# ligengen/EgoGen

Measured on AMD Instinct MI355X. Metric: PPO env-steps/sec (512 parallel SMPL-X agents), higher is better.
Workload: dtype f32 (blend GEMM: shape/template columns as 2-term bf16 splits, pose correctives as one fp16 product, fp32 accumulate); PPO update products on 2-term bf16 splits; rollout policy layers on 2-term bf16 splits

## Files before the change

egogen_amd/_lib.py:

```python
from __future__ import annotations

import ctypes as C
import os

_HERE = os.path.dirname(os.path.abspath(__file__))
LIB_PATH = os.path.join(_HERE, "libegogen_hip.so")

c_float_p = C.POINTER(C.c_float)
c_int_p = C.POINTER(C.c_int32)


class EgxError(RuntimeError):
    pass


class BodyModelHost(C.Structure):
    _fields_ = [
        ("num_verts", C.c_int),
        ("v_template_host", C.c_void_p), ("shapedirs_host", C.c_void_p), ("posedirs_host", C.c_void_p),
        ("J_regressor_host", C.c_void_p), ("parents_host", C.c_void_p), ("lbs_weights_host", C.c_void_p),
        ("hand_comps_l_host", C.c_void_p), ("hand_comps_r_host", C.c_void_p),
        ("hand_mean_l_host", C.c_void_p), ("hand_mean_r_host", C.c_void_p),
        ("extra_vids_host", C.c_void_p), ("lmk_vids_host", C.c_void_p), ("lmk_bary_host", C.c_void_p),
        ("num_markers", C.c_int), ("marker_vids_host", C.c_void_p),
# ... 220 lines not shown
    "egx_sample_action": (C.c_int, [C.c_void_p, C.c_void_p, C.c_void_p, C.c_float, C.c_float, C.c_int, C.c_int, C.c_void_p,
                                    C.c_void_p, C.c_void_p]),
    "egx_gae": (C.c_int, [C.c_void_p, C.c_void_p, C.c_void_p, C.c_int, C.c_int, C.c_double, C.c_double, C.c_void_p,
                          C.c_void_p, C.c_void_p]),
    "egx_ppo_loss": (C.c_int, [C.c_void_p] * 9 + [C.c_float] * 6 + [C.c_int] + [C.c_void_p] * 5),
    "egx_gru_pointwise_bwd": (C.c_int, [C.c_void_p, C.c_void_p, C.c_void_p, C.c_void_p, C.c_int, C.c_int, C.c_void_p, C.c_void_p,
                                        C.c_void_p, C.c_void_p]),
    "egx_ppo_loss_packed": (C.c_int, [C.c_void_p] * 8 + [C.c_float] * 6 + [C.c_int] + [C.c_void_p] * 4),
    "egx_lbs_set_blend_mode": (C.c_int, [C.c_int]),
    "egx_lbs_get_blend_mode": (C.c_int, []),
    "egx_lbs_set_wave_tile": (C.c_int, [C.c_int]),
    "egx_lbs_get_wave_tile": (C.c_int, []),
    "egx_lbs_set_fix_queue_capacity": (C.c_int, [C.c_int]),
    "egx_lbs_fix_stats": (C.c_int, [C.c_void_p, C.c_void_p, C.c_int, C.POINTER(C.c_int32)]),
    "egx_gather_rows": (C.c_int, [C.c_void_p, C.c_int, C.c_int, C.c_void_p, C.c_void_p, C.c_void_p, C.c_void_p]),
    "egx_adv_stats": (C.c_int, [C.c_void_p, C.c_int, C.c_void_p, C.c_void_p]),
    "egx_track_episode": (C.c_int, [C.c_void_p, C.c_void_p, C.c_int, C.c_void_p, C.c_void_p, C.c_void_p, C.c_void_p]),
    "egx_rollout_store": (C.c_int, [C.c_void_p] * 6 + [C.c_int] + [C.c_void_p] * 10),
    "egx_adamw_workspace_floats": (C.c_size_t, []),
    "egx_adamw_clip_step": (C.c_int, [C.c_void_p, C.c_void_p, C.c_void_p, C.c_void_p, C.c_size_t, C.c_size_t, C.c_float] + [C.c_double] * 5 +
                            [C.c_void_p, C.c_void_p, C.c_void_p]),
    "egx_policy_set_precision": (C.c_int, [C.c_int]),
    "egx_policy_get_precision": (C.c_int, []),
    "egx_act_fwd": (C.c_int, [C.c_void_p, C.c_void_p, C.c_void_p, C.c_int, C.c_int, C.c_int, C.c_float, C.c_void_p]),
    "egx_act_bwd_colsum": (C.c_int, [C.c_void_p, C.c_void_p, C.c_void_p, C.c_void_p, C.c_int, C.c_int, C.c_int, C.c_float,
                                     C.c_void_p]),
    "egx_profile_next_lbs": (C.c_int, [C.c_void_p, C.c_void_p]),
    "egx_event_create": (C.c_int, [C.POINTER(C.c_void_p)]),
    "egx_event_destroy": (C.c_int, [C.c_void_p]),
    "egx_event_elapsed_ms": (C.c_int, [C.c_void_p, C.c_void_p, C.POINTER(C.c_float)]),
    "egx_policy_train_create": (C.c_int, [C.POINTER(PolicyWeights), C.POINTER(PolicyGrads), C.c_int, C.POINTER(C.c_void_p)]),
    "egx_policy_train_destroy": (None, [C.c_void_p]),
    "egx_policy_train_refresh": (C.c_int, [C.c_void_p, C.c_void_p]),
    "egx_policy_train_packed": (C.c_int, [C.c_void_p, C.POINTER(PolicyPacked3)]),
    "egx_policy_train_bind": (C.c_int, [C.c_void_p, C.c_void_p, C.c_void_p]),
    "egx_policy_train_step": (C.c_int, [C.c_void_p] * 9 + [C.c_float] * 6 + [C.c_void_p, C.c_void_p]),
    "egx_policy_train_step_heads": (C.c_int, [C.c_void_p] * 9 + [C.c_float] * 6 + [C.c_void_p, C.c_void_p]),
    "egx_policy_train_step_encoders": (C.c_int, [C.c_void_p, C.c_void_p]),
    "egx_policy_train_set_precision": (C.c_int, [C.c_void_p, C.c_int]),
    "egx_policy_train_dense3_launches": (C.c_int, [C.c_void_p]),
    "egx_policy_train_head": (C.c_int, [C.c_void_p, C.POINTER(UpdateHead), C.c_void_p]),
    "egx_policy_train_step_cursor": (C.c_int, [C.c_void_p, C.POINTER(UpdateHead), C.c_void_p] + [C.c_float] * 6 + [C.c_void_p]),
    "egx_policy_train_step_heads_cursor": (C.c_int, [C.c_void_p, C.POINTER(UpdateHead), C.c_void_p] + [C.c_float] * 6 + [C.c_void_p]),
    "egx_adamw_clip_step_cursor": (C.c_int, [C.c_void_p, C.c_void_p, C.c_void_p, C.c_void_p, C.c_size_t, C.c_size_t, C.c_float] +
                                   [C.c_double] * 5 + [C.c_void_p, C.c_void_p, C.c_void_p, C.c_void_p]),
    "egx_policy_train_bind_flat": (C.c_int, [C.c_void_p, C.c_void_p, C.c_size_t]),
# ... 57 lines not shown
```

egogen_amd/csrc/body_model.hip:

```cpp
#include <algorithm>
#include <atomic>
#include <cstdlib>

#include "egx_sdf.h"
#include "lbs_pack.h"

static thread_local hipEvent_t g_prof_start = nullptr, g_prof_stop = nullptr;
extern "C" int egx_profile_next_lbs(void* start_event, void* stop_event) {
  g_prof_start = static_cast<hipEvent_t>(start_event);
  g_prof_stop = static_cast<hipEvent_t>(stop_event);
  return EGX_OK;
}

namespace {
constexpr int BODY_PAD = 256;
}

__global__ void egx_gather_kernel(const float* __restrict__ picked, int B, int NP, int M,
                                  const int* __restrict__ marker_slot, const int* __restrict__ extra_slot,
                                  const int* __restrict__ lmk_slot, const float* __restrict__ lmk_bary,
                                  float* __restrict__ out_joints, float* __restrict__ out_markers) {
  const int b = blockIdx.x;
  const float* pk = picked + (size_t)b * NP * 3;
  for (int i = threadIdx.x; i < M + NEXTRA + NLMK; i += blockDim.x) {
    if (i < M) {
      if (out_markers) {
        const float* s = pk + marker_slot[i] * 3;
        float* o = out_markers + ((size_t)b * M + i) * 3;
        o[0] = s[0]; o[1] = s[1]; o[2] = s[2];
      }
    } else if (out_joints) {
      float* o = out_joints + ((size_t)b * EGX_NUM_JOINTS_OUT + NJ + (i - M)) * 3;
      if (i < M + NEXTRA) {
        const float* s = pk + extra_slot[i - M] * 3;
        o[0] = s[0]; o[1] = s[1]; o[2] = s[2];
      } else {
        const int l = i - M - NEXTRA;
        float acc[3] = {0.f, 0.f, 0.f};
        for (int k = 0; k < 3; ++k) {
          const float* s = pk + lmk_slot[l * 3 + k] * 3;
          const float w = lmk_bary[l * 3 + k];
          acc[0] += s[0] * w; acc[1] += s[1] * w; acc[2] += s[2] * w;
        }
        o[0] = acc[0]; o[1] = acc[1]; o[2] = acc[2];
      }
    }
  }
}

extern "C" int egx_body_model_create(const egx_body_model_host* d, egx_body_model** out) {
  EGX_REQUIRE(d && out, "null argument");
  LbsPacked p;
  if (int rc = lbs_pack_model(d, &p)) return rc;
  auto* m = new egx_body_model();
  static_cast<LbsModelDims&>(*m) = p;
  auto u16 = [](bf16x8** dptr) { return reinterpret_cast<unsigned short**>(dptr); };
  int rc = EGX_OK;
  if ((rc = egx_upload(&m->cull_E, p.cull_E)) || (rc = egx_upload(&m->cull_D0, p.cull_D0)) || (rc = egx_upload(u16(&m->dirs3), p.dirs3)) ||
      (rc = egx_upload(u16(&m->dirs4), p.dirs4)) || (rc = egx_upload(u16(&m->skinW), p.skinW)) || (rc = egx_upload(&m->skin_ks_off, p.skin_ks_off)) ||
      (rc = egx_upload(&m->dirs_rm, p.dirs_rm)) || (rc = egx_upload(&m->vorig, p.perm)) || (rc = egx_upload(&m->pick_tiles, p.pick_tiles)) ||
      (rc = egx_upload(&m->sdf_tiles, p.sdf_tiles)) || (rc = egx_upload(&m->dirs, p.dirs)) || (rc = egx_upload(&m->tj_off, p.tj_off)) ||
      (rc = egx_upload(&m->tj_idx, p.tj_idx)) || (rc = egx_upload(&m->tj_w, p.tj_w)) || (rc = egx_upload(&m->pick_slot, p.pick_slot)) ||
      (rc = egx_upload(&m->vflags, p.vflags)) || (rc = egx_upload(&m->pc, p.pc)) || (rc = egx_upload(&m->marker_slot, p.marker_slot)) ||
      (rc = egx_upload(&m->extra_slot, p.extra_slot)) || (rc = egx_upload(&m->lmk_slot, p.lmk_slot)) ||
      (rc = egx_upload(&m->lmk_bary, p.lmk_bary))) {
    egx_body_model_destroy(m);
    return rc;
  }
  *out = m;
  return EGX_OK;
}
// ... 211 lines not shown
  int* order = cull ? reinterpret_cast<int*>(ws + wl.order) : nullptr;
  int* flags = reinterpret_cast<int*>(ws + wl.flags);
  int* items = reinterpret_cast<int*>(ws + wl.items);
  int* counts = reinterpret_cast<int*>(ws + wl.counts);
  float* fvec = cull ? reinterpret_cast<float*>(ws + wl.fvec) : nullptr;
  float* jpos = cull ? reinterpret_cast<float*>(ws + wl.jpos) : nullptr;
  if (cull) lbs_launch_cull_order(m, xb, R0, T0, sd, mips, B, fpa, nbg_all, order, flags, counts, stream);
  const SdfSceneDev* scene_tab = ms ? set->table : nullptr;
  const int n_scenes = ms ? set->S : 0;
  LbsPoseArgs a;
  a.pc = m->pc; a.xb = xb; a.betas = betas; a.B = B; a.fpa = fpa; a.A4 = A4; a.out_joints = out_joints; a.joints_ld = EGX_NUM_JOINTS_OUT;
  if (split3) a.feat3 = reinterpret_cast<unsigned short*>(feat); else a.feat = feat;
  a.template_lo_feat = (split3 && mode >= 2) ? 1.f : 0.f;
  a.feat4 = (split3 && mode == 3) ? feat4 : nullptr;
  a.zero_counts = sdf ? out_pene_count : nullptr;
  a.agent_of_slot = order; a.fvec = fvec; a.jpos = jpos; a.Bp = (int)wl.Bp;
  a.fix_e = fix ? reinterpret_cast<float*>(ws + wl.fix_e) : nullptr;
  a.skinB = fix ? reinterpret_cast<unsigned short*>(ws + wl.skinB) : nullptr;
  a.fix_stats = reinterpret_cast<int*>(ws + wl.fix_stats); a.cinit = reinterpret_cast<f32x4*>(ws + wl.cinit);
  a.R0 = R0; a.T0 = T0; a.sdf = sd; a.scenes = scene_tab; a.agent_scene = agent_scene; a.n_scenes = n_scenes;
  lbs_launch_pose(ms, stream, a);
  if (cull)
    lbs_launch_cull_items(m, fvec, jpos, (int)wl.Bp, order, B, fpa, nbg_all, R0, T0, sd, mips, flags, items, wl.items_stride, counts, stream);
  if (out_verts || need_picks || sdf) {
    LbsParams p;
    p.dirs = m->dirs; p.tj_off = m->tj_off; p.tj_idx = m->tj_idx; p.tj_w = m->tj_w; p.pick_slot = m->pick_slot;
    p.dirs3 = m->dirs3; p.feat3 = reinterpret_cast<const bf16x8*>(feat);
    p.dirs4 = m->dirs4; p.feat4 = reinterpret_cast<const bf16x8*>(feat4);
    p.vorig = m->vorig;
    p.vflags = m->vflags; p.feat = reinterpret_cast<const f32x4*>(feat); p.A4 = A4; p.xb = xb;
    p.B = B; p.V = m->V; p.NVT = m->NVT; p.NW = m->NW; p.NP = m->NP; p.fpa = fpa;
    p.nbg = egx_ceil_div(B, BODY_PAD);
#ifdef EGX_LBS_DEVELOPMENT
    {
      const char* e = getenv("EGX_LBS_DBG");
      p.dbg = e ? atoi(e) : 0;
    }
#else
    p.dbg = 0;
#endif
    p.verts = out_verts; p.picked = picked; p.R0 = R0; p.T0 = T0; p.pene = out_pene_count;
    p.agent_of_slot = order; p.items = cull ? items : nullptr; p.item_counts = counts; p.items_stride = wl.items_stride;
    p.tiles = out_verts ? nullptr : (sdf ? m->sdf_tiles : m->pick_tiles);
    p.n_tiles = out_verts ? m->NVT : (sdf ? m->n_sdf_tiles : m->n_pick_tiles);
    p.n_precise = sdf ? (m->sdf_lead_picks ? m->n_pick_tiles : m->n_sdf_tiles) : m->n_pick_tiles;
#ifdef EGX_LBS_DEVELOPMENT
    if (const char* e = getenv("EGX_LBS_PRECISE")) p.n_precise = atoi(e);
#endif
    p.sdf = sd;
    p.fix_e = reinterpret_cast<const float*>(ws + wl.fix_e);
    p.fix_stats = reinterpret_cast<int*>(ws + wl.fix_stats);
    p.skinW = m->skinW; p.skin_ks_off = m->skin_ks_off;
    p.fixq = reinterpret_cast<int2*>(ws + wl.fixq); p.fixq_cap = g_fixq_cap.load() > 0 ? g_fixq_cap.load() : LBS_FIXQ_CAP;
    p.dirs_rm = m->dirs_rm; p.pc = m->pc; p.betas = betas;
    p.skinB = reinterpret_cast<const bf16x8*>(ws + wl.skinB); p.cinit = reinterpret_cast<const f32x4*>(ws + wl.cinit);
    p.sdf_aux = ms ? nullptr : aux;
    p.scenes = scene_tab; p.agent_scene = agent_scene; p.n_scenes = n_scenes;
    p.bg_block = 3;
#ifdef EGX_LBS_DEVELOPMENT
    if (const char* e = getenv("EGX_LBS_BG_BLOCK")) p.bg_block = atoi(e);
#endif
    hipEvent_t ev0 = g_prof_start, ev1 = g_prof_stop;
    g_prof_start = g_prof_stop = nullptr;
    if (ev0) EGX_HIP_CHECK(hipEventRecord(ev0, stream));
    if (int rc = split3 ? lbs_launch_fused3(p, mode, sdf != nullptr, ms, wave_tile(), stream) : lbs_launch_fused(p, sdf != nullptr, ms, stream))
      return rc;
    if (fix) lbs_launch_fix(p, ms, stream);
    if (ev1) EGX_HIP_CHECK(hipEventRecord(ev1, stream));
  }
  if (need_picks)
    hipLaunchKernelGGL(egx_gather_kernel, dim3(B), dim3(256), 0, stream, picked, B, m->NP, m->M, m->marker_slot,
                       m->extra_slot, m->lmk_slot, m->lmk_bary, out_joints, out_markers);
  EGX_HIP_CHECK(hipGetLastError());
  return EGX_OK;
}

extern "C" int egx_lbs_forward(const egx_body_model* m, const float* xb, const float* betas, int B, int fpa,
                               float* out_verts, float* out_joints, float* out_markers, const egx_sdf_grid* sdf,
                               const float* R0, const float* T0, int32_t* out_pene_count, void* workspace,
                               size_t workspace_bytes, void* stream) {
  return lbs_forward_launch(m, xb, betas, B, fpa, out_verts, out_joints, out_markers, sdf, nullptr, nullptr, R0, T0, out_pene_count,
                            workspace, workspace_bytes, stream);
}

extern "C" int egx_lbs_forward_scenes(const egx_body_model* m, const float* xb, const float* betas, int B, int fpa,
                                      float* out_verts, float* out_joints, float* out_markers, const egx_sdf_scene_set* scenes,
                                      const int32_t* agent_scene, const float* R0, const float* T0, int32_t* out_pene_count,
                                      void* workspace, size_t workspace_bytes, void* stream) {
  EGX_REQUIRE(scenes && agent_scene && out_pene_count, "a scene-set call needs the set, agent_scene and out_pene_count");
  if (scenes->S == 1) {
    if (int rc = lbs_forward_launch(m, xb, betas, B, fpa, out_verts, out_joints, out_markers, &scenes->dims, nullptr, nullptr, R0, T0,
                                    out_pene_count, workspace, workspace_bytes, stream))
      return rc;
    hipLaunchKernelGGL(egx_lbs_scene_mark_kernel, dim3(egx_ceil_div(B, 256)), dim3(256), 0, static_cast<hipStream_t>(stream), agent_scene,
                       1, B, fpa, out_pene_count);
// ... 7 lines not shown
```

egogen_amd/csrc/egx_common.h:

```cpp
#pragma once
#include <hip/hip_runtime.h>
#include <stdint.h>
#include <stdio.h>
#include <string>
#include <vector>

#include "../../include/egogen_hip.h"

typedef float f32x16 __attribute__((ext_vector_type(16)));
typedef float f32x4 __attribute__((ext_vector_type(4)));
typedef short bf16x8 __attribute__((ext_vector_type(8)));
__host__ __device__ inline unsigned short egx_bf16_rne(float x) {
  union { float f; unsigned u; } c;
  c.f = x;
  if ((c.u & 0x7fffffffu) > 0x7f800000u) return (unsigned short)((c.u >> 16) | 0x40u);
  return (unsigned short)((c.u + 0x7fffu + ((c.u >> 16) & 1u)) >> 16);
}
__host__ __device__ inline float egx_bf16_to_f32(unsigned short h) {
  union { float f; unsigned u; } c;
  c.u = (unsigned)h << 16;
  return c.f;
}


void egx_set_error(const std::string& msg);

#define EGX_HIP_CHECK(expr)                                                                   \
  do {                                                                                        \
    hipError_t _e = (expr);                                                                   \
    if (_e != hipSuccess) {                                                                   \
      egx_set_error(std::string(#expr) + ": " + hipGetErrorString(_e));                       \
      return EGX_ERR_HIP;                                                                     \
    }                                                                                         \
  } while (0)

#define EGX_REQUIRE(cond, msg)                                                                \
  do {                                                                                        \
    if (!(cond)) {                                                                            \
      egx_set_error(std::string("argument check failed: ") + #cond + " - " + (msg));          \
      return EGX_ERR_ARG;                                                                     \
    }                                                                                         \
  } while (0)

static inline int egx_ceil_div(int a, int b) { return (a + b - 1) / b; }
static inline size_t egx_align_up(size_t x, size_t a) { return (x + a - 1) / a * a; }

template <typename T>
static int egx_upload(T** dptr, const std::vector<T>& h) {
// ... 18 lines not shown
```

egogen_amd/csrc/egx_nets.h:

```cpp
#pragma once
#include "egx_common.h"
#include "egx_frame.h"

struct EgxSeg {
  const float* p;
  int w, ld;
};

int egx_launch_linear(hipStream_t st, int M, int N, const EgxSeg* segs, int nseg, const float* W, const float* b,
                      int act, float slope, const float* res, int ldr, float* out, int ldo);
int egx_launch_gru_pointwise(hipStream_t st, const float* gi, const float* gh, const float* hprev, int ldh, float* hout,
                             int ldo, int M, int H);
int egx_launch_cont6d_to_aa(hipStream_t st, const float* xb6, int n, float* out, int ldo);
int egx_launch_posenc(hipStream_t st, const float* dist, const float* time, int A, float* out);

void egx_launch_frame_scan(hipStream_t st, float* y, const float* x_last, int x_ld, int A, int width, int T);

struct D3Pack {
  const float* src;
  int R, K, ld, col0;
  void* dst;
  int S_total, s0;
  int transpose = 0;
};
void egx_launch_pack3(hipStream_t st, const D3Pack* jobs, int njobs);

struct D3Plain {
  const bf16x8* A = nullptr;
  int SA = 0, sa0 = 0;
  const bf16x8* B = nullptr;
  int S = 0;
  const float* bias = nullptr;
  const float* res = nullptr;
  int ldr = 0;
  float* out = nullptr;
  int ldo = 0;
  bf16x8* out3 = nullptr;
  int S3 = 0, s30 = 0;
  int M = 0, N = 0, act = 0;
  float slope = 0.f;
  int batches = 1;
  size_t batch_strideA = 0, batch_stride3 = 0;
  int batch_rows_out = 0;
  int prec = 0;
  float* out_act = nullptr;
  int ldact = 0;
  const float* dact = nullptr;
  int lddact = 0, dact_code = 0;
// ... 135 lines not shown
```

egogen_amd/csrc/lbs.h:

```cpp
#pragma once
#include <mutex>

#include "egx_common.h"
#include "egx_sdf.h"

namespace {

constexpr int NJ = EGX_NUM_JOINTS;
constexpr int KACT = 10 + 51 * 9;
constexpr int KDIM = EGX_BLEND_K;
constexpr int KSTEPS = KDIM / 2;
constexpr int KGROUPS = KSTEPS / 4;
static_assert(KGROUPS >= 2, "the operand ring preloads two k-groups");
constexpr int KS3 = 30;
__host__ __device__ inline void egx_bf16_split3(float x, unsigned short* h) {
  h[0] = egx_bf16_rne(x);
  const float r1 = x - egx_bf16_to_f32(h[0]);
  h[1] = egx_bf16_rne(r1);
  const float r2 = r1 - egx_bf16_to_f32(h[1]);
  h[2] = egx_bf16_rne(r2);
}
constexpr int M4_BASE_PIECES = 96, M4_FEAT_PIECES = 32;
constexpr int M4_FKS = 4;
__host__ __device__ inline int egx_m4_feat_piece(int s, int pl) { return s == 0 ? pl : (s <= 28 ? s + 1 : 30 + pl); }
// ... 226 lines not shown
struct LbsPoseArgs {
  const PoseConsts* pc = nullptr;
  const float *xb = nullptr, *betas = nullptr, *R0 = nullptr, *T0 = nullptr;
  int B = 0, fpa = 0, joints_ld = 0, Bp = 0;
  float *feat = nullptr, *out_joints = nullptr, *fvec = nullptr, *jpos = nullptr, *fix_e = nullptr;
  unsigned short *feat3 = nullptr, *feat4 = nullptr, *skinB = nullptr;
  f32x4 *A4 = nullptr, *cinit = nullptr;
  int *zero_counts = nullptr, *fix_stats = nullptr;
  const int* agent_of_slot = nullptr;
  float template_lo_feat = 0.f;
  SdfDev sdf = {};
  const SdfSceneDev* scenes = nullptr;
  const int* agent_scene = nullptr;
  int n_scenes = 0;
};
void lbs_launch_pose(bool ms, hipStream_t stream, const LbsPoseArgs& a);
void lbs_launch_cull_order(const egx_body_model* m, const float* xb, const float* R0, const float* T0, const SdfDev& sd, const float* mips,
                           int B, int fpa, int nbg_all, int* order, int* flags, int* counts, hipStream_t stream);
void lbs_launch_cull_items(const egx_body_model* m, const float* fvec, const float* jpos, int Bp, const int* order, int B, int fpa,
                           int nbg_all, const float* R0, const float* T0, const SdfDev& sd, const float* mips, int* flags, int* items,
                           int items_stride, int* counts, hipStream_t stream);
int lbs_launch_fused(const LbsParams& p, bool do_sdf, bool ms, hipStream_t stream);
int lbs_launch_fused3(const LbsParams& p, int mode, bool do_sdf, bool ms, int forced_tile, hipStream_t stream);
void lbs_launch_fix(const LbsParams& p, bool ms, hipStream_t stream);
```

egogen_amd/csrc/lbs_fix.hip:

```cpp
#include "lbs_epilogue.h"

constexpr int LBS_FIX_BLOCKS = 1024;
static_assert((LBS_FIX_BLOCKS * 4) % LBS_FIX_NQ == 0, "waves of the fix-up kernel per sub-queue");
template <bool MS>
__global__ __launch_bounds__(256) void egx_lbs_fix_kernel(LbsParams p) {
  const int lane = threadIdx.x & 63;
  const int wave = blockIdx.x * 4 + (threadIdx.x >> 6), n_waves = gridDim.x * 4;
  const int sq = wave % LBS_FIX_NQ;
  const int count = min(p.fix_stats[LBS_FIX_CNT0 + 32 * sq], p.fixq_cap);
  for (int i = wave / LBS_FIX_NQ; i < count; i += n_waves / LBS_FIX_NQ) {
    const int2 e = p.fixq[(size_t)sq * p.fixq_cap + i];
    if (e.x < 0) continue;
    const int vt = e.x >> 5, row = e.x & 31, slot = e.y;
    const int j_lo = p.tj_off[vt], JT = p.tj_off[vt + 1] - j_lo;
    const float sv = lbs_fix_one<true, MS>(p, lane, vt, row, slot, JT, p.tj_idx + j_lo, p.tj_w + (size_t)j_lo * 32);
    if (lane == 0 && sv < 0.f) {
      const int body = p.agent_of_slot ? p.agent_of_slot[slot / p.fpa] * p.fpa + slot % p.fpa : slot;
      atomicAdd(p.pene + body, 1);
    }
  }
}

void lbs_launch_fix(const LbsParams& p, bool ms, hipStream_t stream) {
  hipLaunchKernelGGL(ms ? egx_lbs_fix_kernel<true> : egx_lbs_fix_kernel<false>, dim3(LBS_FIX_BLOCKS), dim3(256), 0, stream, p);
}
```

egogen_amd/csrc/pack3.hip:

```cpp
#include "d3.h"

struct D3PackJob {
  const float* src;
  int R, K, ld, col0;
  bf16x8* dst;
  int S_total, s0;
  int transpose;
};
struct D3PackJobs {
  D3PackJob j0, j1, j2, j3;
  int end0, end1, end2;
};

__global__ __launch_bounds__(256) void egx_pack3_kernel(D3PackJobs jobs) {
  int frag = blockIdx.x * 4 + (threadIdx.x >> 6);
  const int which = frag < jobs.end0 ? 0 : (frag < jobs.end1 ? 1 : (frag < jobs.end2 ? 2 : 3));
  const D3PackJob& j = which == 0 ? jobs.j0 : (which == 1 ? jobs.j1 : (which == 2 ? jobs.j2 : jobs.j3));
  frag -= which == 0 ? 0 : (which == 1 ? jobs.end0 : (which == 2 ? jobs.end1 : jobs.end2));
  const int lane = threadIdx.x & 63;
  const int RT = 2 * ((j.R + 31) >> 5), S = (j.K + 31) >> 5;
  if (!j.src || frag >= RT * S) return;
  const int rt = frag / S, s = frag % S;
  const int row = rt * 16 + (lane & 15), k0 = s * 32 + 8 * (lane >> 4);
  float x[8];
  if (!j.transpose) {
#pragma unroll
    for (int e = 0; e < 8; ++e) x[e] = (row < j.R && k0 + e < j.K) ? j.src[(size_t)row * j.ld + j.col0 + k0 + e] : 0.f;
  } else {
#pragma unroll
    for (int e = 0; e < 8; ++e) x[e] = (row < j.R && k0 + e < j.K) ? j.src[(size_t)(k0 + e) * j.ld + j.col0 + row] : 0.f;
  }
  bf16x8 pl[3];
  d3_split(x, pl);
  bf16x8* o = j.dst + ((size_t)rt * j.S_total + j.s0 + s) * 3 * 64 + lane;
#pragma unroll
  for (int p = 0; p < 3; ++p) o[p * 64] = pl[p];
}

void egx_launch_pack3(hipStream_t st, const D3Pack* jobs, int njobs) {
  D3PackJobs J;
  D3PackJob* dst[4] = {&J.j0, &J.j1, &J.j2, &J.j3};
  int frags[4] = {0, 0, 0, 0};
  for (int i = 0; i < 4; ++i) {
    D3PackJob& d = *dst[i];
    if (i < njobs) {
      d.src = jobs[i].src; d.R = jobs[i].R; d.K = jobs[i].K; d.ld = jobs[i].ld; d.col0 = jobs[i].col0;
      d.dst = static_cast<bf16x8*>(jobs[i].dst); d.S_total = jobs[i].S_total; d.s0 = jobs[i].s0;
      d.transpose = jobs[i].transpose;
      frags[i] = (int)d3_img_frags(d.R, d.K);
    } else {
      d.src = nullptr; d.R = d.K = d.ld = d.col0 = d.S_total = d.s0 = d.transpose = 0; d.dst = nullptr;
    }
  }
  J.end0 = frags[0]; J.end1 = J.end0 + frags[1]; J.end2 = J.end1 + frags[2];
  const int total = J.end2 + frags[3];
  hipLaunchKernelGGL(egx_pack3_kernel, dim3(egx_ceil_div(total, 4)), dim3(256), 0, st, J);
}

__global__ __launch_bounds__(256) void egx_posenc3_kernel(const float* __restrict__ dist, const float* __restrict__ time, int n,
                                                          float* __restrict__ out, int ld, bf16x8* __restrict__ out3, int S3, int s0,
                                                          bf16x8* __restrict__ out3T, int S3T, int col0T, float* __restrict__ zero6) {
  if (zero6 && blockIdx.x == 0 && threadIdx.x < 6) zero6[threadIdx.x] = 0.f;
  egx_posenc3_role(dist, time, n, out, ld, out3, S3, s0, out3T, S3T, col0T, (int)blockIdx.x, EgxRowsIdentity());
}
void egx_launch_posenc3(hipStream_t st, const float* dist, const float* time, int n, float* out, int ld, void* out3, int S3, int s0,
                        void* out3T, int S3T, int col0T, float* zero6) {
  const int frags = 2 * egx_ceil_div(n, 32) * 4 + (out3T ? 8 * egx_ceil_div(n, 32) : 0);
  hipLaunchKernelGGL(egx_posenc3_kernel, dim3(egx_ceil_div(frags, 4)), dim3(256), 0, st, dist, time, n, out, ld,
                     static_cast<bf16x8*>(out3), S3, s0, static_cast<bf16x8*>(out3T), S3T, col0T, zero6);
}

extern "C" size_t egx_pack3_bytes(int num_rows, int num_cols) {
  if (num_rows <= 0 || num_cols <= 0) return 0;
  return d3_img_frags(num_rows, num_cols) * D3_FRAG_BYTES;
}
extern "C" int egx_pack3(const float* src, int num_rows, int num_cols, int src_ld, int src_col0, void* dst, int dst_ksteps,
                         int dst_kstep0, void* stream) {
  EGX_REQUIRE(src && dst && num_rows > 0 && num_cols > 0 && src_ld >= src_col0 + num_cols, "bad arguments");
  const int S = egx_ceil_div(num_cols, 32);
// ... 7 lines not shown
```

egogen_amd/csrc/prior.hip:

```cpp
#include <algorithm>
#include <atomic>
#include "d3.h"

namespace {
constexpr int H = 256, ZD = 128, MK = 201, T_PRED = 18;

struct Carver {
  char* base;
  size_t off = 0, cap;
  Carver(void* p, size_t c) : base(static_cast<char*>(p)), cap(c) {}
  float* take(size_t nfloat) {
    float* r = reinterpret_cast<float*>(base + off);
    off = egx_align_up(off + nfloat * sizeof(float), 256);
    return r;
  }
};
size_t carve_bytes(std::initializer_list<size_t> nfloats) {
  size_t off = 0;
  for (size_t n : nfloats) off = egx_align_up(off + n * sizeof(float), 256);
  return off;
}
}

constexpr size_t FRAG_FLOATS = D3_FRAG_BYTES / sizeof(float);
constexpr int S_MK = 7, S_H = 8, S_HZ = 12, S_512 = 16;

extern "C" size_t egx_sample_prior_workspace_bytes(int A) {
  if (A <= 0) return 0;
  const size_t a = A;
  const size_t rt = d3_img_tiles(A);
  return carve_bytes({rt * S_MK * FRAG_FLOATS, rt * S_MK * FRAG_FLOATS, rt * S_HZ * FRAG_FLOATS,
                      rt * S_H * FRAG_FLOATS, rt * S_512 * FRAG_FLOATS, rt * S_H * FRAG_FLOATS,
                      rt * S_H * FRAG_FLOATS, rt * S_H * FRAG_FLOATS, T_PRED * rt * S_H * FRAG_FLOATS,
                      a * 3 * H, a * 3 * H, a * H, a * H, a * H});
}

static int sample_prior_packed(const egx_prior_weights* w, const float* x0, const float* x1, int x_ld, const float* z, int A,
                               float* out_Y, void* workspace, size_t workspace_bytes, hipStream_t st) {
  const egx_prior_packed3& P = *w->packed3;
  Carver cv(workspace, workspace_bytes);
  const size_t rt = d3_img_tiles(A);
  auto take3 = [&](size_t ksteps) { return reinterpret_cast<bf16x8*>(cv.take(rt * ksteps * FRAG_FLOATS)); };
  bf16x8* x0p = take3(S_MK);
  bf16x8* x1p = take3(S_MK);
// ... 21 lines not shown
    g.h_out = hBf; g.ldo = H; g.h_out3 = hB3; g.S3 = S_H;
    egx_launch_gru3(st, g);
    g.Ai = x1p;
    g.Ah = hB3; g.SAh = S_H; g.Bh = B3(P.x_enc_w_hh); g.Sh = S_H; g.h_prev = hBf; g.ldh = H;
    g.h_out = nullptr; g.h_out3 = hz3; g.S3 = S_HZ;
    egx_launch_gru3(st, g);
  }
  {
    D3Plain l0, gc;
    l0.M = A; l0.N = 512; l0.A = hz3; l0.SA = S_HZ; l0.S = S_H; l0.B = B3(P.drnn_w[0]); l0.bias = w->drnn_b[0]; l0.act = 1;
    l0.out3 = t512; l0.S3 = S_512;
    gc.M = A; gc.N = 3 * H; gc.A = hz3; gc.SA = S_HZ; gc.S = S_HZ; gc.B = B3(P.d_rnn_w_hz); gc.bias = w->d_rnn_b_ih;
    gc.out = gconst; gc.ldo = 3 * H;
    egx_launch_dense3_pair(st, l0, gc);
    D3Plain l1;
    l1.M = A; l1.N = H; l1.A = t512; l1.SA = S_512; l1.S = S_512; l1.B = B3(P.drnn_w[1]); l1.bias = w->drnn_b[1]; l1.act = 1;
    l1.out3 = t256; l1.S3 = S_H;
    egx_launch_dense3(st, l1);
    D3Plain l2;
    l2.M = A; l2.N = H; l2.A = t256; l2.SA = S_H; l2.S = S_H; l2.B = B3(P.drnn_w[2]); l2.bias = w->drnn_b[2]; l2.act = 1;
    l2.out = hf[0]; l2.ldo = H; l2.out3 = h3[0]; l2.S3 = S_H;
    egx_launch_dense3(st, l2);
  }
  int cur = 0;
  for (int i = 0; i < T_PRED; ++i) {
    D3Gru g;
    g.M = A; g.H = H;
    if (i == 0) {
      g.Ai = x1p; g.SAi = S_MK; g.Bi = B3(P.d_rnn_w_y); g.Si = S_MK; g.gi_in = gconst;
    } else {
      g.Ai = hfc_all + (size_t)(i - 1) * hfc_stride; g.SAi = S_H; g.Bi = B3(P.d_comb_w); g.Si = S_H; g.bias_i = w->d_comb_b; g.gi_in = gi;
    }
    g.gi_out = gi;
    g.Ah = h3[cur]; g.SAh = S_H; g.Bh = B3(P.d_rnn_w_hh); g.Sh = S_H; g.bias_h = w->d_rnn_b_hh;
    g.h_prev = hf[cur]; g.ldh = H; g.h_out = hf[cur ^ 1]; g.ldo = H; g.h_out3 = h3[cur ^ 1]; g.S3 = S_H;
    egx_launch_gru3(st, g);
    cur ^= 1;
    D3Plain m0;
    m0.M = A; m0.N = 512; m0.A = h3[cur]; m0.SA = S_H; m0.S = S_H; m0.B = B3(P.d_mlp_w[0]); m0.bias = w->d_mlp_b[0]; m0.act = 1;
    m0.out3 = t512; m0.S3 = S_512;
    egx_launch_dense3(st, m0);
    D3Plain m1;
    m1.M = A; m1.N = H; m1.A = t512; m1.SA = S_512; m1.S = S_512; m1.B = B3(P.d_mlp_w[1]); m1.bias = w->d_mlp_b[1]; m1.act = 1;
    m1.out3 = hfc_all + (size_t)i * hfc_stride; m1.S3 = S_H;
    egx_launch_dense3(st, m1);
  }
  {
    D3Plain o;
    o.M = A; o.N = MK; o.A = hfc_all; o.SA = S_H; o.S = S_H; o.B = B3(P.d_out_w); o.bias = w->d_out_b;
    o.out = out_Y; o.ldo = MK; o.batches = T_PRED; o.batch_strideA = hfc_stride; o.batch_rows_out = A;
    egx_launch_dense3(st, o);
    egx_launch_frame_scan(st, out_Y, x1, x_ld, A, MK, T_PRED);
  }
  return EGX_OK;
}

extern "C" int egx_sample_prior(const egx_prior_weights* w, const float* x0, const float* x1, int x_ld,
                                const float* betas, const float* z, int A, float* out_Y, float* out_Yb,
                                void* workspace, size_t workspace_bytes, void* stream_) {
  EGX_REQUIRE(w && x0 && x1 && betas && z && out_Y && out_Yb, "null argument");
  EGX_REQUIRE(A > 0 && x_ld >= MK, "bad sizes");
  if (!workspace || workspace_bytes < egx_sample_prior_workspace_bytes(A)) {
    egx_set_error("egx_sample_prior: workspace too small");
    return EGX_ERR_WORKSPACE;
  }
  hipStream_t st = static_cast<hipStream_t>(stream_);
  const int M = A * T_PRED;
  EGX_REQUIRE(w->packed3, "egx_sample_prior needs the packed weight images (egx_prior_weights.packed3, built with egx_pack3)");
  EGX_REQUIRE(w->d_comb_w && w->d_comb_b, "egx_sample_prior needs the folded output layer (d_comb_w / d_comb_b)");
  const egx_prior_packed3& P = *w->packed3;
  EGX_REQUIRE(P.reg_in_m && P.reg_in_xb && P.reg_in_betas && P.reg_blk && P.reg_out && P.reg_blk_b, "packed regressor weights missing");
  int rc = sample_prior_packed(w, x0, x1, x_ld, z, A, out_Y, workspace, workspace_bytes, st);
  if (rc) return rc;
  RegWeights3 r3;
// ... 39 lines not shown
  const size_t rt = d3_img_tiles(n), m = n;
  auto take3 = [&](size_t ksteps) { return reinterpret_cast<bf16x8*>(cv.take(rt * ksteps * FRAG_FLOATS)); };
  bf16x8* s0p = take3(PS_ST);
  bf16x8* s1p = take3(PS_ST);
  bf16x8* e0p = take3(PS_EGO);
  bf16x8* e1p = take3(PS_EGO);
  bf16x8* hx1 = take3(PS_HD);
  bf16x8* he1 = take3(PS_HD);
  bf16x8* cat3 = take3(PS_CAT);
  bf16x8* a1 = take3(PS_CAT);
  bf16x8* a2 = take3(PS_CAT);
  bf16x8* c1 = take3(PS_CAT);
  bf16x8* c2 = take3(PS_CAT);
  float* hx1f = cv.take(m * 512);
  float* he1f = cv.take(m * 512);
  float* catf = cv.take(m * 1152);
  float* a2f = cv.take(m * 1152);
  float* c2f = cv.take(m * 1152);
  constexpr int HD = 512;
  auto B3 = [](const void* p) { return static_cast<const bf16x8*>(p); };
  {
    const D3Pack jobs[4] = {{state, n, 402, 804, 0, s0p, PS_ST, 0}, {state, n, 402, 804, 402, s1p, PS_ST, 0},
                            {ego, n, 32, 64, 0, e0p, PS_EGO, 0}, {ego, n, 32, 64, 32, e1p, PS_EGO, 0}};
    egx_launch_pack3(st, jobs, 4);
  }
  egx_launch_posenc3(st, dist, time, n, catf + 2 * HD, 1152, cat3, PS_CAT, 2 * PS_HD);
  {
    struct Enc { const bf16x8 *x0, *x1; int Sx; const void *w_ih, *w_hh; const float *b_ih, *b_hh; bf16x8* h1; float* h1f; int col0, s30; };
    const Enc enc[2] = {{s0p, s1p, PS_ST, P.x_enc_w_ih, P.x_enc_w_hh, w->x_enc_b_ih, w->x_enc_b_hh, hx1, hx1f, 0, 0},
                        {e0p, e1p, PS_EGO, P.ego_enc_w_ih, P.ego_enc_w_hh, w->ego_enc_b_ih, w->ego_enc_b_hh, he1, he1f, HD, PS_HD}};
    D3Gru g[2];
    for (int e = 0; e < 2; ++e) {
      const Enc& E = enc[e];
      g[e].M = n; g[e].H = HD; g[e].prec = prec;
      g[e].Ai = E.x0; g[e].SAi = E.Sx; g[e].Bi = B3(E.w_ih); g[e].Si = E.Sx; g[e].bias_i = E.b_ih; g[e].bias_h = E.b_hh;
      g[e].h_out = E.h1f; g[e].ldo = HD; g[e].h_out3 = E.h1; g[e].S3 = PS_HD;
    }
    egx_launch_gru3_pair(st, g[0], g[1]);
    for (int e = 0; e < 2; ++e) {
      const Enc& E = enc[e];
      g[e].Ai = E.x1;
      g[e].Ah = E.h1; g[e].SAh = PS_HD; g[e].Bh = B3(E.w_hh); g[e].Sh = PS_HD; g[e].h_prev = E.h1f; g[e].ldh = HD;
      g[e].h_out = catf + E.col0; g[e].ldo = 1152; g[e].h_out3 = cat3; g[e].S3 = PS_CAT; g[e].s30 = E.s30;
    }
    egx_launch_gru3_pair(st, g[0], g[1]);
  }
  const float slope = 0.01f;
  const bool do_a = out_mu != nullptr, do_c = out_value != nullptr;
  auto layer = [&](const bf16x8* xin, const void* W, const float* b, const float* res, float* outf, bf16x8* out3) {
// ... 65 lines not shown
```

include/egogen_hip.h:

```cpp
#ifndef EGOGEN_HIP_H
#define EGOGEN_HIP_H

#include <stddef.h>
#include <stdint.h>

#ifdef __cplusplus
extern "C" {
#endif

#define EGX_OK 0
#define EGX_ERR_ARG (-1)
#define EGX_ERR_HIP (-2)
#define EGX_ERR_WORKSPACE (-3)
#define EGX_ERR_CONVERGENCE (-4)

#define EGX_NUM_JOINTS 55
#define EGX_NUM_JOINTS_OUT 127
#define EGX_XB_DIM 93
#define EGX_MAX_CANDIDATES 256
#define EGX_MAX_BEAM 32
#define EGX_MAX_OBSTACLES 32
#define EGX_MAX_GROUP 32
#define EGX_MAX_SWEEPS 8
#define EGX_MAX_WAYPOINTS 16
// ... 244 lines not shown
  const int64_t* perm;
  const int32_t* cursor;
  int max_cursor;
  int num_src_rows;
  const float *state, *egosensing, *dist, *time;
  const float *act, *adv, *ret, *logp_old;
  float *act_c, *adv_c, *ret_c, *logp_old_c;
  float* stats;
  int compute_stats;
  float* log;
} egx_update_head;
int egx_policy_train_head(egx_policy_train* h, const egx_update_head* head, void* stream);
int egx_policy_train_step_cursor(egx_policy_train* h, const egx_update_head* head, const float* scale, float adv_eps,
                                 float min_logvar, float max_logvar, float eps_clip, float vf_coef, float ent_coef, void* stream);
int egx_policy_train_step_heads_cursor(egx_policy_train* h, const egx_update_head* head, const float* scale, float adv_eps,
                                       float min_logvar, float max_logvar, float eps_clip, float vf_coef, float ent_coef,
                                       void* stream);
int egx_policy_train_set_precision(egx_policy_train* h, int prec);
int egx_policy_train_dense3_launches(const egx_policy_train* h);

int egx_policy_set_precision(int bf16);
int egx_policy_get_precision(void);

size_t egx_policy_workspace_bytes(int num_rows);

int egx_policy_forward(const egx_policy_weights* w, const float* state, const float* egosensing, const float* dist,
                       const float* time, int num_rows, float* out_mu, float* out_logvar, float* out_value,
                       void* workspace, size_t workspace_bytes, void* stream);

typedef struct egx_vposer_weights {
  const float *fc1_w, *fc1_b;
  const float *fc2_w, *fc2_b;
  const float *mu_w, *mu_b;
  const void *fc1_w3, *fc2_w3, *mu_w3;
} egx_vposer_weights;

size_t egx_vposer_workspace_bytes(int num_rows);
int egx_vposer_encode(const egx_vposer_weights* w, const float* x, int x_ld, int num_rows, float* out,
                      void* workspace, size_t workspace_bytes, void* stream);

typedef struct egx_env_config {
  float reproj_factor, goal_thresh, pene_thres;
  float weight_skate, weight_floor, weight_face_target, weight_look_target, weight_success, weight_target_dist,
      weight_pene, weight_vp;
  int max_depth;
  int scene_kind;
// ... 326 lines not shown
```

Before: 200,400.

## Fold gather, posenc and prior output layer into neighbouring rollout kernels

```diff
diff --git a/egogen_amd/_lib.py b/egogen_amd/_lib.py
--- a/egogen_amd/_lib.py
+++ b/egogen_amd/_lib.py
@@ -266,6 +266,9 @@
                             [C.c_void_p, C.c_void_p, C.c_void_p]),
     "egx_policy_set_precision": (C.c_int, [C.c_int]),
     "egx_policy_get_precision": (C.c_int, []),
+    "egx_rollout_set_fold": (C.c_int, [C.c_int]),
+    "egx_rollout_get_fold": (C.c_int, []),
+    "egx_rollout_fold_taken": (C.c_int, []),
     "egx_act_fwd": (C.c_int, [C.c_void_p, C.c_void_p, C.c_void_p, C.c_int, C.c_int, C.c_int, C.c_float, C.c_void_p]),
     "egx_act_bwd_colsum": (C.c_int, [C.c_void_p, C.c_void_p, C.c_void_p, C.c_void_p, C.c_int, C.c_int, C.c_int, C.c_float,
                                      C.c_void_p]),
diff --git a/egogen_amd/csrc/body_model.hip b/egogen_amd/csrc/body_model.hip
--- a/egogen_amd/csrc/body_model.hip
+++ b/egogen_amd/csrc/body_model.hip
@@ -16,37 +16,7 @@
 constexpr int BODY_PAD = 256;
 }
 
-__global__ void egx_gather_kernel(const float* __restrict__ picked, int B, int NP, int M,
-                                  const int* __restrict__ marker_slot, const int* __restrict__ extra_slot,
-                                  const int* __restrict__ lmk_slot, const float* __restrict__ lmk_bary,
-                                  float* __restrict__ out_joints, float* __restrict__ out_markers) {
-  const int b = blockIdx.x;
-  const float* pk = picked + (size_t)b * NP * 3;
-  for (int i = threadIdx.x; i < M + NEXTRA + NLMK; i += blockDim.x) {
-    if (i < M) {
-      if (out_markers) {
-        const float* s = pk + marker_slot[i] * 3;
-        float* o = out_markers + ((size_t)b * M + i) * 3;
-        o[0] = s[0]; o[1] = s[1]; o[2] = s[2];
-      }
-    } else if (out_joints) {
-      float* o = out_joints + ((size_t)b * EGX_NUM_JOINTS_OUT + NJ + (i - M)) * 3;
-      if (i < M + NEXTRA) {
-        const float* s = pk + extra_slot[i - M] * 3;
-        o[0] = s[0]; o[1] = s[1]; o[2] = s[2];
-      } else {
-        const int l = i - M - NEXTRA;
-        float acc[3] = {0.f, 0.f, 0.f};
-        for (int k = 0; k < 3; ++k) {
-          const float* s = pk + lmk_slot[l * 3 + k] * 3;
-          const float w = lmk_bary[l * 3 + k];
-          acc[0] += s[0] * w; acc[1] += s[1] * w; acc[2] += s[2] * w;
-        }
-        o[0] = acc[0]; o[1] = acc[1]; o[2] = acc[2];
-      }
-    }
-  }
-}
+__global__ void egx_gather_kernel(LbsGatherArgs g) { lbs_gather_role(g, (int)blockIdx.x); }
 
 extern "C" int egx_body_model_create(const egx_body_model_host* d, egx_body_model** out) {
   EGX_REQUIRE(d && out, "null argument");
@@ -304,6 +274,11 @@
   lbs_launch_pose(ms, stream, a);
   if (cull)
     lbs_launch_cull_items(m, fvec, jpos, (int)wl.Bp, order, B, fpa, nbg_all, R0, T0, sd, mips, flags, items, wl.items_stride, counts, stream);
+  LbsGatherArgs ga;
+  ga.picked = picked; ga.B = B; ga.NP = m->NP; ga.M = m->M; ga.marker_slot = m->marker_slot; ga.extra_slot = m->extra_slot;
+  ga.lmk_slot = m->lmk_slot; ga.lmk_bary = m->lmk_bary; ga.out_joints = out_joints; ga.out_markers = out_markers;
+  const bool fold_gather = need_picks && fix && (egx_rollout_get_fold() & EGX_FOLD_GATHER) != 0;
+  egx_rollout_fold_note(EGX_FOLD_GATHER, fold_gather);
   if (out_verts || need_picks || sdf) {
     LbsParams p;
     p.dirs = m->dirs; p.tj_off = m->tj_off; p.tj_idx = m->tj_idx; p.tj_w = m->tj_w; p.pick_slot = m->pick_slot;
@@ -347,12 +322,10 @@
     if (ev0) EGX_HIP_CHECK(hipEventRecord(ev0, stream));
     if (int rc = split3 ? lbs_launch_fused3(p, mode, sdf != nullptr, ms, wave_tile(), stream) : lbs_launch_fused(p, sdf != nullptr, ms, stream))
       return rc;
-    if (fix) lbs_launch_fix(p, ms, stream);
+    if (fix) lbs_launch_fix(p, ms, stream, fold_gather ? &ga : nullptr);
     if (ev1) EGX_HIP_CHECK(hipEventRecord(ev1, stream));
   }
-  if (need_picks)
-    hipLaunchKernelGGL(egx_gather_kernel, dim3(B), dim3(256), 0, stream, picked, B, m->NP, m->M, m->marker_slot,
-                       m->extra_slot, m->lmk_slot, m->lmk_bary, out_joints, out_markers);
+  if (need_picks && !fold_gather) hipLaunchKernelGGL(egx_gather_kernel, dim3(B), dim3(256), 0, stream, ga);
   EGX_HIP_CHECK(hipGetLastError());
   return EGX_OK;
 }
diff --git a/egogen_amd/csrc/egx_common.h b/egogen_amd/csrc/egx_common.h
--- a/egogen_amd/csrc/egx_common.h
+++ b/egogen_amd/csrc/egx_common.h
@@ -24,6 +24,7 @@
 
 
 void egx_set_error(const std::string& msg);
+void egx_rollout_fold_note(int bit, bool taken);
 
 #define EGX_HIP_CHECK(expr)                                                                   \
   do {                                                                                        \
diff --git a/egogen_amd/csrc/egx_nets.h b/egogen_amd/csrc/egx_nets.h
--- a/egogen_amd/csrc/egx_nets.h
+++ b/egogen_amd/csrc/egx_nets.h
@@ -24,6 +24,8 @@
   int transpose = 0;
 };
 void egx_launch_pack3(hipStream_t st, const D3Pack* jobs, int njobs);
+void egx_launch_pack3_posenc(hipStream_t st, const D3Pack* jobs, int njobs, const float* dist, const float* time, int n, float* out,
+                             int ld, void* out3, int S3, int s0);
 
 struct D3Plain {
   const bf16x8* A = nullptr;
diff --git a/egogen_amd/csrc/lbs.h b/egogen_amd/csrc/lbs.h
--- a/egogen_amd/csrc/lbs.h
+++ b/egogen_amd/csrc/lbs.h
@@ -272,4 +272,47 @@
                            int items_stride, int* counts, hipStream_t stream);
 int lbs_launch_fused(const LbsParams& p, bool do_sdf, bool ms, hipStream_t stream);
 int lbs_launch_fused3(const LbsParams& p, int mode, bool do_sdf, bool ms, int forced_tile, hipStream_t stream);
-void lbs_launch_fix(const LbsParams& p, bool ms, hipStream_t stream);
+struct LbsGatherArgs {
+  const float* picked = nullptr;
+  int B = 0, NP = 0, M = 0;
+  const int *marker_slot = nullptr, *extra_slot = nullptr, *lmk_slot = nullptr;
+  const float* lmk_bary = nullptr;
+  float *out_joints = nullptr, *out_markers = nullptr;
+};
+#if defined(__HIPCC__)
+__device__ __forceinline__ void lbs_gather_role(const LbsGatherArgs& g, int b) {
+  const float* __restrict__ pk = g.picked + (size_t)b * g.NP * 3;
+  const int* __restrict__ marker_slot = g.marker_slot;
+  const int* __restrict__ extra_slot = g.extra_slot;
+  const int* __restrict__ lmk_slot = g.lmk_slot;
+  const float* __restrict__ lmk_bary = g.lmk_bary;
+  float* __restrict__ out_joints = g.out_joints;
+  float* __restrict__ out_markers = g.out_markers;
+  const int M = g.M;
+  for (int i = threadIdx.x; i < M + NEXTRA + NLMK; i += blockDim.x) {
+    if (i < M) {
+      if (out_markers) {
+        const float* s = pk + marker_slot[i] * 3;
+        float* o = out_markers + ((size_t)b * M + i) * 3;
+        o[0] = s[0]; o[1] = s[1]; o[2] = s[2];
+      }
+    } else if (out_joints) {
+      float* o = out_joints + ((size_t)b * EGX_NUM_JOINTS_OUT + NJ + (i - M)) * 3;
+      if (i < M + NEXTRA) {
+        const float* s = pk + extra_slot[i - M] * 3;
+        o[0] = s[0]; o[1] = s[1]; o[2] = s[2];
+      } else {
+        const int l = i - M - NEXTRA;
+        float acc[3] = {0.f, 0.f, 0.f};
+        for (int k = 0; k < 3; ++k) {
+          const float* s = pk + lmk_slot[l * 3 + k] * 3;
+          const float w = lmk_bary[l * 3 + k];
+          acc[0] += s[0] * w; acc[1] += s[1] * w; acc[2] += s[2] * w;
+        }
+        o[0] = acc[0]; o[1] = acc[1]; o[2] = acc[2];
+      }
+    }
+  }
+}
+#endif
+void lbs_launch_fix(const LbsParams& p, bool ms, hipStream_t stream, const LbsGatherArgs* gather = nullptr);
diff --git a/egogen_amd/csrc/lbs_fix.hip b/egogen_amd/csrc/lbs_fix.hip
--- a/egogen_amd/csrc/lbs_fix.hip
+++ b/egogen_amd/csrc/lbs_fix.hip
@@ -2,10 +2,16 @@
 
 constexpr int LBS_FIX_BLOCKS = 1024;
 static_assert((LBS_FIX_BLOCKS * 4) % LBS_FIX_NQ == 0, "waves of the fix-up kernel per sub-queue");
-template <bool MS>
-__global__ __launch_bounds__(256) void egx_lbs_fix_kernel(LbsParams p) {
+template <bool MS, bool GATHER>
+__global__ __launch_bounds__(256) void egx_lbs_fix_kernel(LbsParams p, LbsGatherArgs g) {
+  if constexpr (GATHER) {
+    if ((int)blockIdx.x >= LBS_FIX_BLOCKS) {
+      lbs_gather_role(g, (int)blockIdx.x - LBS_FIX_BLOCKS);
+      return;
+    }
+  }
   const int lane = threadIdx.x & 63;
-  const int wave = blockIdx.x * 4 + (threadIdx.x >> 6), n_waves = gridDim.x * 4;
+  const int wave = blockIdx.x * 4 + (threadIdx.x >> 6), n_waves = LBS_FIX_BLOCKS * 4;
   const int sq = wave % LBS_FIX_NQ;
   const int count = min(p.fix_stats[LBS_FIX_CNT0 + 32 * sq], p.fixq_cap);
   for (int i = wave / LBS_FIX_NQ; i < count; i += n_waves / LBS_FIX_NQ) {
@@ -21,6 +27,12 @@
   }
 }
 
-void lbs_launch_fix(const LbsParams& p, bool ms, hipStream_t stream) {
-  hipLaunchKernelGGL(ms ? egx_lbs_fix_kernel<true> : egx_lbs_fix_kernel<false>, dim3(LBS_FIX_BLOCKS), dim3(256), 0, stream, p);
+void lbs_launch_fix(const LbsParams& p, bool ms, hipStream_t stream, const LbsGatherArgs* gather) {
+  if (gather) {
+    hipLaunchKernelGGL((ms ? egx_lbs_fix_kernel<true, true> : egx_lbs_fix_kernel<false, true>), dim3(LBS_FIX_BLOCKS + gather->B), dim3(256), 0,
+                       stream, p, *gather);
+  } else {
+    hipLaunchKernelGGL((ms ? egx_lbs_fix_kernel<true, false> : egx_lbs_fix_kernel<false, false>), dim3(LBS_FIX_BLOCKS), dim3(256), 0, stream, p,
+                       LbsGatherArgs{});
+  }
 }
diff --git a/egogen_amd/csrc/pack3.hip b/egogen_amd/csrc/pack3.hip
--- a/egogen_amd/csrc/pack3.hip
+++ b/egogen_amd/csrc/pack3.hip
@@ -11,8 +11,23 @@
   D3PackJob j0, j1, j2, j3;
   int end0, end1, end2;
 };
+struct D3PackPosenc {
+  const float *dist, *time;
+  int n;
+  float* out;
+  int ld;
+  bf16x8* out3;
+  int S3, s0, block0;
+};
 
-__global__ __launch_bounds__(256) void egx_pack3_kernel(D3PackJobs jobs) {
+template <bool PE>
+__global__ __launch_bounds__(256) void egx_pack3_kernel(D3PackJobs jobs, D3PackPosenc pe) {
+  if constexpr (PE) {
+    if ((int)blockIdx.x >= pe.block0) {
+      egx_posenc3_role(pe.dist, pe.time, pe.n, pe.out, pe.ld, pe.out3, pe.S3, pe.s0, nullptr, 0, 0, (int)blockIdx.x - pe.block0, EgxRowsIdentity());
+      return;
+    }
+  }
   int frag = blockIdx.x * 4 + (threadIdx.x >> 6);
   const int which = frag < jobs.end0 ? 0 : (frag < jobs.end1 ? 1 : (frag < jobs.end2 ? 2 : 3));
   const D3PackJob& j = which == 0 ? jobs.j0 : (which == 1 ? jobs.j1 : (which == 2 ? jobs.j2 : jobs.j3));
@@ -37,7 +52,7 @@
   for (int p = 0; p < 3; ++p) o[p * 64] = pl[p];
 }
 
-void egx_launch_pack3(hipStream_t st, const D3Pack* jobs, int njobs) {
+static void d3_launch_pack3(hipStream_t st, const D3Pack* jobs, int njobs, const D3PackPosenc* posenc) {
   D3PackJobs J;
   D3PackJob* dst[4] = {&J.j0, &J.j1, &J.j2, &J.j3};
   int frags[4] = {0, 0, 0, 0};
@@ -54,7 +69,20 @@
   }
   J.end0 = frags[0]; J.end1 = J.end0 + frags[1]; J.end2 = J.end1 + frags[2];
   const int total = J.end2 + frags[3];
-  hipLaunchKernelGGL(egx_pack3_kernel, dim3(egx_ceil_div(total, 4)), dim3(256), 0, st, J);
+  const int blocks = egx_ceil_div(total, 4);
+  if (posenc) {
+    D3PackPosenc pe = *posenc;
+    pe.block0 = blocks;
+    hipLaunchKernelGGL(egx_pack3_kernel<true>, dim3(blocks + egx_ceil_div(2 * egx_ceil_div(pe.n, 32) * 4, 4)), dim3(256), 0, st, J, pe);
+  } else {
+    hipLaunchKernelGGL(egx_pack3_kernel<false>, dim3(blocks), dim3(256), 0, st, J, D3PackPosenc{});
+  }
+}
+void egx_launch_pack3(hipStream_t st, const D3Pack* jobs, int njobs) { d3_launch_pack3(st, jobs, njobs, nullptr); }
+void egx_launch_pack3_posenc(hipStream_t st, const D3Pack* jobs, int njobs, const float* dist, const float* time, int n, float* out,
+                             int ld, void* out3, int S3, int s0) {
+  const D3PackPosenc pe{dist, time, n, out, ld, static_cast<bf16x8*>(out3), S3, s0, 0};
+  d3_launch_pack3(st, jobs, njobs, &pe);
 }
 
 __global__ __launch_bounds__(256) void egx_posenc3_kernel(const float* __restrict__ dist, const float* __restrict__ time, int n,
diff --git a/egogen_amd/csrc/prior.hip b/egogen_amd/csrc/prior.hip
--- a/egogen_amd/csrc/prior.hip
+++ b/egogen_amd/csrc/prior.hip
@@ -20,6 +20,20 @@
   for (size_t n : nfloats) off = egx_align_up(off + n * sizeof(float), 256);
   return off;
 }
+std::atomic<int> g_rollout_fold{EGX_FOLD_ALL};
+std::atomic<int> g_rollout_fold_taken{0};
+}
+
+extern "C" int egx_rollout_set_fold(int mask) {
+  EGX_REQUIRE(mask >= 0 && mask <= EGX_FOLD_ALL, "fold mask: bits EGX_FOLD_PRIOR_OUT | EGX_FOLD_POSENC | EGX_FOLD_GATHER");
+  g_rollout_fold.store(mask);
+  return EGX_OK;
+}
+extern "C" int egx_rollout_get_fold(void) { return g_rollout_fold.load(); }
+extern "C" int egx_rollout_fold_taken(void) { return g_rollout_fold_taken.load(); }
+void egx_rollout_fold_note(int bit, bool taken) {
+  if (taken) g_rollout_fold_taken.fetch_or(bit);
+  else g_rollout_fold_taken.fetch_and(~bit);
 }
 
 constexpr size_t FRAG_FLOATS = D3_FRAG_BYTES / sizeof(float);
@@ -87,6 +101,29 @@
     l2.out = hf[0]; l2.ldo = H; l2.out3 = h3[0]; l2.S3 = S_H;
     egx_launch_dense3(st, l2);
   }
+  auto out_layer = [&](int i) {
+    D3Plain o;
+    o.M = A; o.N = MK; o.A = hfc_all + (size_t)i * hfc_stride; o.SA = S_H; o.S = S_H; o.B = B3(P.d_out_w); o.bias = w->d_out_b;
+    o.out = out_Y + (size_t)i * A * MK; o.ldo = MK;
+    o.res = i == 0 ? x1 : out_Y + (size_t)(i - 1) * A * MK; o.ldr = i == 0 ? x_ld : MK;
+    return o;
+  };
+  D3Plain out_all;
+  out_all.M = A; out_all.N = MK; out_all.A = hfc_all; out_all.SA = S_H; out_all.S = S_H; out_all.B = B3(P.d_out_w); out_all.bias = w->d_out_b;
+  out_all.out = out_Y; out_all.ldo = MK; out_all.batches = T_PRED; out_all.batch_strideA = hfc_stride; out_all.batch_rows_out = A;
+  auto mlp0 = [&](const bf16x8* h) {
+    D3Plain m0;
+    m0.M = A; m0.N = 512; m0.A = h; m0.SA = S_H; m0.S = S_H; m0.B = B3(P.d_mlp_w[0]); m0.bias = w->d_mlp_b[0]; m0.act = 1;
+    m0.out3 = t512; m0.S3 = S_512;
+    return m0;
+  };
+  bool fold_out = (g_rollout_fold.load() & EGX_FOLD_PRIOR_OUT) != 0;
+  if (fold_out) {
+    const D3Plain pair[2] = {mlp0(h3[0]), out_layer(0)};
+    const int cfg = egx_dense3_config(&out_all, 1);
+    fold_out = egx_dense3_config(pair, 2) == cfg && egx_dense3_config(&pair[0], 1) == cfg && egx_dense3_config(&pair[1], 1) == cfg;
+  }
+  egx_rollout_fold_note(EGX_FOLD_PRIOR_OUT, fold_out);
   int cur = 0;
   for (int i = 0; i < T_PRED; ++i) {
     D3Gru g;
@@ -101,20 +138,17 @@
     g.h_prev = hf[cur]; g.ldh = H; g.h_out = hf[cur ^ 1]; g.ldo = H; g.h_out3 = h3[cur ^ 1]; g.S3 = S_H;
     egx_launch_gru3(st, g);
     cur ^= 1;
-    D3Plain m0;
-    m0.M = A; m0.N = 512; m0.A = h3[cur]; m0.SA = S_H; m0.S = S_H; m0.B = B3(P.d_mlp_w[0]); m0.bias = w->d_mlp_b[0]; m0.act = 1;
-    m0.out3 = t512; m0.S3 = S_512;
-    egx_launch_dense3(st, m0);
+    if (fold_out && i > 0) egx_launch_dense3_pair(st, mlp0(h3[cur]), out_layer(i - 1));
+    else egx_launch_dense3(st, mlp0(h3[cur]));
     D3Plain m1;
     m1.M = A; m1.N = H; m1.A = t512; m1.SA = S_512; m1.S = S_512; m1.B = B3(P.d_mlp_w[1]); m1.bias = w->d_mlp_b[1]; m1.act = 1;
     m1.out3 = hfc_all + (size_t)i * hfc_stride; m1.S3 = S_H;
     egx_launch_dense3(st, m1);
   }
-  {
-    D3Plain o;
-    o.M = A; o.N = MK; o.A = hfc_all; o.SA = S_H; o.S = S_H; o.B = B3(P.d_out_w); o.bias = w->d_out_b;
-    o.out = out_Y; o.ldo = MK; o.batches = T_PRED; o.batch_strideA = hfc_stride; o.batch_rows_out = A;
-    egx_launch_dense3(st, o);
+  if (fold_out) {
+    egx_launch_dense3(st, out_layer(T_PRED - 1));
+  } else {
+    egx_launch_dense3(st, out_all);
     egx_launch_frame_scan(st, out_Y, x1, x_ld, A, MK, T_PRED);
   }
   return EGX_OK;
@@ -200,9 +234,15 @@
   {
     const D3Pack jobs[4] = {{state, n, 402, 804, 0, s0p, PS_ST, 0}, {state, n, 402, 804, 402, s1p, PS_ST, 0},
                             {ego, n, 32, 64, 0, e0p, PS_EGO, 0}, {ego, n, 32, 64, 32, e1p, PS_EGO, 0}};
-    egx_launch_pack3(st, jobs, 4);
-  }
-  egx_launch_posenc3(st, dist, time, n, catf + 2 * HD, 1152, cat3, PS_CAT, 2 * PS_HD);
+    const bool fold_pe = (g_rollout_fold.load() & EGX_FOLD_POSENC) != 0;
+    egx_rollout_fold_note(EGX_FOLD_POSENC, fold_pe);
+    if (fold_pe) {
+      egx_launch_pack3_posenc(st, jobs, 4, dist, time, n, catf + 2 * HD, 1152, cat3, PS_CAT, 2 * PS_HD);
+    } else {
+      egx_launch_pack3(st, jobs, 4);
+      egx_launch_posenc3(st, dist, time, n, catf + 2 * HD, 1152, cat3, PS_CAT, 2 * PS_HD);
+    }
+  }
   {
     struct Enc { const bf16x8 *x0, *x1; int Sx; const void *w_ih, *w_hh; const float *b_ih, *b_hh; bf16x8* h1; float* h1f; int col0, s30; };
     const Enc enc[2] = {{s0p, s1p, PS_ST, P.x_enc_w_ih, P.x_enc_w_hh, w->x_enc_b_ih, w->x_enc_b_hh, hx1, hx1f, 0, 0},
diff --git a/include/egogen_hip.h b/include/egogen_hip.h
--- a/include/egogen_hip.h
+++ b/include/egogen_hip.h
@@ -290,6 +290,11 @@
 int egx_policy_set_precision(int bf16);
 int egx_policy_get_precision(void);
 
+enum { EGX_FOLD_PRIOR_OUT = 1, EGX_FOLD_POSENC = 2, EGX_FOLD_GATHER = 4, EGX_FOLD_ALL = 7 };
+int egx_rollout_set_fold(int mask);
+int egx_rollout_get_fold(void);
+int egx_rollout_fold_taken(void);
+
 size_t egx_policy_workspace_bytes(int num_rows);
 
 int egx_policy_forward(const egx_policy_weights* w, const float* state, const float* egosensing, const float* dist,
```

New measurement: 200,400 (median of 2 runs). About the same (-0.0%).
